# mayataka/robotoc

Measured on AMD Instinct MI355X. Metric: riccati_sweeps_per_sec, higher is better.
Workload: dtype f64; 1 GPU; anymal_trot_N40 (nv=18,nu=12, 47 grids: 2 lifts + 2 impacts, switching constraints ns=6), 4096 DISTINCT OCP instances per GPU (randomised stage data and dx0), backward+forward Riccati sweep; per_gpu_batch=4096, stages=47, parallelism=instances sharded, dp1

## Files before the change

### robotoc_amd/csrc/riccati_backward_rv.hpp

```cpp
#pragma once
#include "riccati_backward.hpp"

namespace rtoc {

template <int NV, int NU>
struct RvCfg {
  static constexpr int NX = 2 * NV;
  static constexpr int T = (NX + 15) / 16;
  static constexpr int LDP = lds_ld(NX);
  static constexpr int KG = (NX + 3) / 4;
  static constexpr int KSU = (NU + 3) / 4;
  static constexpr int SCOL = NX - 16 * (T - 1);
  static constexpr int G0 = NV / 4;
  static constexpr int GS = 4 * (T - 1) + SCOL / 4;
  static constexpr bool STRIP4 = (SCOL == 4);
  static constexpr bool OK = (NX + NU == 16 * T) && (NX % 4 == 0) && (NU % 4 == 0) && (SCOL % 4 == 0) && (SCOL >= 1) &&
                             ((NV * NU) % 2 == 0) && (LDP % 2 == 0);
  static constexpr int HL = LDP / 2;
  static constexpr int NCH_A = NX * HL;
  static constexpr int PA = (NCH_A + 63) / 64;
  static constexpr int OFF_A = 0;
  static constexpr int OFF_ST = NX * LDP;
  static constexpr int CB = NV * NU / 2, CG = NU * NU / 2;
  static constexpr int pad8(int n) { return (n + 7) & ~7; }
// ... 22 lines not shown
#else
  return *p;
#endif
}
__device__ __forceinline__ void rv_st(double* p, double v) {
#if RTOC_RV_NT
  __builtin_nontemporal_store(v, p);
#else
  *p = v;
#endif
}
constexpr int RV_DMA_AUX = RTOC_RV_NT ? 2 : 0;

template <int N>
__device__ __forceinline__ double dpp_from_right(double v) {
  const int lo = __builtin_amdgcn_update_dpp(0, __double2loint(v), 0x100 + N, 0xF, 0xF, true);
  const int hi = __builtin_amdgcn_update_dpp(0, __double2hiint(v), 0x100 + N, 0xF, 0xF, true);
  return __hiloint2double(hi, lo);
}
template <int N>
__device__ __forceinline__ double dpp_from_left(double v) {
  const int lo = __builtin_amdgcn_update_dpp(0, __double2loint(v), 0x110 + N, 0xF, 0xF, true);
  const int hi = __builtin_amdgcn_update_dpp(0, __double2hiint(v), 0x110 + N, 0xF, 0xF, true);
  return __hiloint2double(hi, lo);
}

constexpr int rv_dpp_ctrl(int from) { return from > 0 ? 0x100 + from : (from < 0 ? 0x110 - from : 0xE4); }
template <int R>
__device__ __forceinline__ double d4_to_c(double d0, double d1) {
  int h[2];
#pragma unroll
  for (int e = 0; e < 2; ++e) {
    const int a0 = e ? __double2hiint(d0) : __double2loint(d0), a1 = e ? __double2hiint(d1) : __double2loint(d1);
    const int x = __builtin_amdgcn_update_dpp(0, a0, rv_dpp_ctrl(4 * R), 0xF, 0x1, true);
    h[e] = __builtin_amdgcn_update_dpp(x, a1, rv_dpp_ctrl(4 * R - 4), 0xF, 0x2, true);
  }
  return __hiloint2double(h[1], h[0]);
}

__host__ __device__ constexpr int rv_tile_row(int T, int n) {
  int k = 0;
  for (int c = 0; c < T; ++c)
    for (int t = c + 1; t < T; ++t) {
      if (k == n) return c;
      ++k;
    }
  return n - k;
}
__host__ __device__ constexpr int rv_tile_col(int T, int n) {
  int k = 0;
  for (int c = 0; c < T; ++c)
    for (int t = c + 1; t < T; ++t) {
      if (k == n) return t;
      ++k;
    }
  return n - k;
}

__device__ __forceinline__ void rv_lds_sync() {
  asm volatile("s_waitcnt lgkmcnt(0)" ::: "memory");
  __builtin_amdgcn_wave_barrier();
}

#ifdef RTOC_ENABLE_PROF
#define RV_PROF(k)                                                                                        \
  do {                                                                                                    \
    if (a.prof && b == 0 && lane0 == 0) a.prof[st * 32 + (k)] = (long long)__builtin_readcyclecounter(); \
  } while (0)
#else
#define RV_PROF(k) do { } while (0)
#endif

template <int NV, int NU, int NS, bool SA, bool STO = false>
__global__ __launch_bounds__(64, 2) void riccati_backward_rv_kernel(BwdArgs a) {
  using C = RvCfg<NV, NU>;
  static_assert(C::OK, "shape does not fill the tiles of the stacked operand");
  constexpr int NP_ = NV - NU;
  static_assert(!SA || (NV % 16 == 2 && C::T == 3 && NP_ > 0 && NP_ <= 8 && NP_ % 2 == 0),
                "structured form: the lane shift of the c-part is NV mod 16 = 2, corner columns in tiles 0 and 1");
  constexpr int NX = C::NX, T = C::T, LDP = C::LDP, KG = C::KG, KSU = C::KSU, SCOL = C::SCOL, G0 = C::G0, GS = C::GS;
  constexpr bool STRIP4 = C::STRIP4 && !STO && RTOC_RV_MERGE_PBT;
  constexpr int RS = SCOL / 4;
  constexpr rtoc_layout SL = StaticLayout<NV, NU, NS>::make();
  constexpr rtoc_record_layout KL = SL.kkt, RL = SL.ric;
  constexpr int VOFF_LX = KL.off[RTOC_KKT_LX] - KL.off[RTOC_KKT_FX], VOFF_LU = KL.off[RTOC_KKT_LU] - KL.off[RTOC_KKT_FX];
  static_assert(VOFF_LX > 0 && VOFF_LU > VOFF_LX && VOFF_LX % 2 == 0 && VOFF_LU % 2 == 0, "Fx, lx, lu lie behind one another in the record");
  static_assert(KL.off[RTOC_KKT_FXX] % 2 == 0 && KL.off[RTOC_KKT_FVU] % 2 == 0 && KL.off[RTOC_KKT_QUU] % 2 == 0 && KL.off[RTOC_KKT_FX] % 2 == 0 &&
                    KL.stride % 2 == 0, "16-byte chunks");
  constexpr int VOFF_FFX = KL.off[RTOC_KKT_FFX] - KL.off[RTOC_KKT_FX], VOFF_HX = KL.off[RTOC_KKT_HX] - KL.off[RTOC_KKT_FX],
                VOFF_HU = KL.off[RTOC_KKT_HU] - KL.off[RTOC_KKT_FX], VOFF_SCAL = KL.off[RTOC_KKT_SCAL] - KL.off[RTOC_KKT_FX];
  static_assert(!STO || (VOFF_FFX > VOFF_LU && VOFF_HX > VOFF_FFX && VOFF_HU > VOFF_HX && VOFF_SCAL > VOFF_HU && VOFF_SCAL % 2 == 0), "fx, hx, hu, scalars behind lu");
  static_assert(!STO || SCOL + 2 < 16, "two more rider lanes in the last column tile");
  static_assert(!STO || SCOL >= 3, "lanes 0..2 of the G product are idle (the controls are shifted by SCOL lanes)");
  constexpr int CB = C::CB, CG = C::CG, CV = STO ? (VOFF_SCAL + 8) / 2 : (VOFF_LU + NU + 1) / 2, NCH_S = CB + CG + CV, PS = (NCH_S + 63) / 64;
  constexpr int ST_BV = C::OFF_ST, ST_G = ST_BV + 2 * CB, ST_FX = ST_G + 2 * CG, ST_LX = ST_FX + VOFF_LX, ST_LU = ST_FX + VOFF_LU;
  constexpr int ST_FFX = ST_FX + VOFF_FFX, ST_HX = ST_FX + VOFF_HX, ST_HU = ST_FX + VOFF_HU, ST_SCAL = ST_FX + VOFF_SCAL;
  constexpr int NSCR = (STO || RTOC_RV_ONE_SCRATCH) ? 1 : 2;
  constexpr int OFF_Y = ST_FX + 2 * CV, OFF_LINV = OFF_Y + C::pad8(NU * NU), OFF_SCR = OFF_LINV + C::pad8(NU), SCR_LD = 17,
                SCR_TILE = C::pad8(16 * SCR_LD), LDS_DOUBLES = OFF_SCR + NSCR * SCR_TILE;
  static_assert(NU * NU <= NSCR * SCR_TILE, "the Cholesky factor is parked in the transpose scratch");
  static_assert(!STO || 2 * C::pad8(NX) + NX <= SCR_TILE, "s | Psi | Phi gathered in the scratch");
  constexpr int OFF_GRID = LDS_DOUBLES, GRID_INTS = 2 * (20 * 1024 / 8 - LDS_DOUBLES);
  static_assert(GRID_INTS >= 64, "room for the grid table");
  static_assert(LDS_DOUBLES * 8 <= 20 * 1024, "eight instances per CU");
  extern __shared__ __attribute__((aligned(16))) double smem[];
  double* const sA = smem + C::OFF_A;
  double* const sBv = smem + ST_BV;
  double* const sG = smem + ST_G;
  double* const sY = smem + OFF_Y;
  double* const scr = smem + OFF_SCR;

  const int b = a.first + (int)blockIdx.x;
  if (b >= a.batch) return;
  const int lane0 = threadIdx.x;
  int lane = lane0 & 63, li = lane & 15, q = lane >> 4;
  const int N = a.nstages - 1;
  const size_t kinst = (size_t)b * a.nstages * KL.stride;
  const size_t rinst = (size_t)b * a.nstages * RL.stride;
  const int hi = a.seg_hi, lo = a.seg_lo;
  unsigned stat = 0;
#ifdef RTOC_RV_DEBUG_MASK
  const int dbg = a.scan_ps_soff;
#define RV_DBG(bit) (dbg & (1 << (bit)))
#else
#define RV_DBG(bit) false
#endif

  auto issue_dma = [&](int stage) {
    const double* kp = a.kkt + kinst + (size_t)stage * KL.stride;
#pragma unroll
    for (int p = 0; p < PS; ++p) {
      const int n = lane + 64 * p;
      const int off = (n < CB) ? (KL.off[RTOC_KKT_FVU] + 2 * n)
                               : ((n < CB + CG) ? (KL.off[RTOC_KKT_QUU] + 2 * (n - CB)) : (KL.off[RTOC_KKT_FX] + 2 * (n - CB - CG)));
      if (64 * (p + 1) <= NCH_S || n < NCH_S)
        __builtin_amdgcn_global_load_lds(kp + off, (lds_ptr_t)(smem + C::OFF_ST + 128 * p), 16, 0, RV_DMA_AUX);
    }
    constexpr int CPP = 64 / C::HL, NPC = (NX + CPP - 1) / CPP;
    const unsigned col0 = (unsigned)lane / C::HL, ch0 = (unsigned)lane - col0 * C::HL;
    const unsigned voff = col0 * NX + ((ch0 < NX / 2) ? 2 * ch0 : 0);
    if (col0 < CPP) {
#pragma unroll
      for (int p = 0; p < NPC; ++p) {
        const double* kpp = kp + KL.off[RTOC_KKT_FXX] + p * CPP * NX;
        if ((p + 1) * CPP <= NX || p * CPP + (int)col0 < NX)
          __builtin_amdgcn_global_load_lds(kpp + voff, (lds_ptr_t)(sA + p * CPP * LDP), 16, 0, RV_DMA_AUX);
      }
    }
  };
  double hq[T][KSU];
  auto issue_hq = [&](int stage) {
    const double* kp = a.kkt + kinst + (size_t)stage * KL.stride + KL.off[RTOC_KKT_QXU];
#pragma unroll
    for (int c = 0; c < T; ++c)
#pragma unroll
      for (int ks = 0; ks < KSU; ++ks) {
        const int x = 16 * c + li, u = 4 * ks + q;
        hq[c][ks] = rv_ld(kp + ((x < NX) ? x : NX - 1) + u * NX);
      }
  };

  d4 pp[T][T];
  double sv[KG];
  {
    const bool term = (hi == N - 1);
    const double* psrc = term ? (a.kkt + kinst + (size_t)N * KL.stride + KL.off[RTOC_KKT_QXX])
                              : (a.ric + rinst + (size_t)(hi + 1) * RL.stride + RL.off[RTOC_RIC_P]);
    const double* ssrc = term ? (a.kkt + kinst + (size_t)N * KL.stride + KL.off[RTOC_KKT_LX])
                              : (a.ric + rinst + (size_t)(hi + 1) * RL.stride + RL.off[RTOC_RIC_S]);
#pragma unroll
    for (int kt = 0; kt < T; ++kt)
#pragma unroll
      for (int mt = 0; mt < T; ++mt)
#pragma unroll
        for (int r = 0; r < 4; ++r) {
          const int i = 16 * kt + 4 * r + q, j = 16 * mt + li;
          const bool ok = i < NX && j < NX;
          const double v = psrc[ok ? i + j * NX : 0];
          pp[kt][mt][r] = ok ? v : 0.0;
        }
#pragma unroll
    for (int g = 0; g < KG; ++g) {
      const double v = ssrc[4 * g + q];
      sv[g] = (li == SCOL) ? (term ? -v : v) : 0.0;
    }
    if (term) {
      double* rr = a.ric + rinst + (size_t)N * RL.stride;
      const d2* s2 = reinterpret_cast<const d2*>(psrc);
      d2* t2 = reinterpret_cast<d2*>(rr + RL.off[RTOC_RIC_P]);
      for (int e = lane; e < NX * NX / 2; e += 64) t2[e] = s2[e];
      if (lane < NX) rr[RL.off[RTOC_RIC_S] + lane] = -ssrc[lane];
    }
  }
  issue_dma(hi);
  int* const sGrid = reinterpret_cast<int*>(smem + OFF_GRID);
  for (int e = lane; e < a.nstages; e += 64)
    sGrid[e] = (a.grid[e].type & 15) | ((a.grid[e].sto != 0) << 4) | ((a.grid[e].sto_next != 0) << 5) | (a.grid[e].dims << 8);
  double sc[5] = {0.0, 0.0, 0.0, 0.0, 0.0};
  auto phase_transition = [&](int pol, bool has_next) __attribute__((always_inline)) {
    double* pr = a.ric + rinst + (size_t)pol * RL.stride;
    const double xi = sc[0], chi = sc[1], rho = sc[2], eta = sc[3], iota = sc[4];
    double isg = 0.0;
    if (has_next) {
      double sgm = xi - 2.0 * chi + rho;
      const double eps = 1.4901161193847656e-08;
      if ((sgm * a.max_dts0) < fabs(eta - iota) || sgm < eps) sgm = fabs(sgm) + fabs(eta - iota) / a.max_dts0;
      isg = 1.0 / sgm;
    }
#pragma unroll
    for (int g = 0; g < KG; ++g) {
      const double v = sv[g];
      const double r1 = dpp_from_right<1>(v), r2 = dpp_from_right<2>(v), l1 = dpp_from_left<1>(v);
      const double d = (li == SCOL) ? (r1 - r2) : (l1 - v);
      double nv = 0.0;
      if (li == SCOL) nv = has_next ? __builtin_fma(isg * (eta - iota), d, v) : v;
      if (li == SCOL + 2) nv = has_next ? __builtin_fma(-isg * (xi - chi), d, l1) : l1;
      sv[g] = (li >= SCOL && li <= SCOL + 2) ? nv : 0.0;
      if (has_next && li == SCOL) pr[RL.off[RTOC_RIC_DTSDX] + 4 * g + q] = -isg * d;
    }
    sc[0] = 0.0, sc[1] = 0.0, sc[3] = 0.0;
    if (has_next) {
      if (lane0 == 0) {
        pr[RL.off[RTOC_RIC_SCAL] + RTOC_RIC_SCAL_DTSDTS] = isg * (xi - chi);
        pr[RL.off[RTOC_RIC_SCAL] + RTOC_RIC_SCAL_DTS0] = -isg * (eta - iota);
      }
      sc[2] = xi - isg * (xi - chi) * (xi - chi);
      sc[4] = eta - isg * (xi - chi) * (eta - iota);
    } else {
      sc[2] = xi;
      sc[4] = eta;
    }
  };
  rv_lds_sync();

  for (int st = hi; st >= lo; --st) {
    lane = lane0;
    asm volatile("" : "+v"(lane));
    lane &= 63;
    li = lane & 15;
    q = lane >> 4;
    const int gword = __builtin_amdgcn_readfirstlane(sGrid[st]);
    const bool impact = (gword & 15) == RTOC_GRID_IMPACT;
    const bool sto = STO && ((gword >> 4) & 1), sto_next = STO && ((gword >> 5) & 1);
    const int ns = impact ? 0 : (gword >> 8);
    const double* kr = a.kkt + kinst + (size_t)st * KL.stride;
    double* rr = a.ric + rinst + (size_t)st * RL.stride;
    if constexpr (STO) {
      const bool next_lift = (__builtin_amdgcn_readfirstlane(sGrid[st + 1]) & 15) == RTOC_GRID_LIFT;
      const bool prev_sto = st > 0 && ((__builtin_amdgcn_readfirstlane(sGrid[st > 0 ? st - 1 : 0]) >> 4) & 1);
      bool do_pt = false;
      int pol = st;
      if (impact) {
        do_pt = prev_sto || sto;
      } else if (next_lift) {
        do_pt = sto || sto_next;
        pol = st + 1;
      }
      if (do_pt) phase_transition(pol, sto_next);
      if (!impact && !sto_next) {
#pragma unroll
        for (int g = 0; g < KG; ++g) sv[g] = (li == SCOL + 2) ? 0.0 : sv[g];
      }
    }
    RV_PROF(0);
    if (st < hi)
      asm volatile("s_waitcnt vmcnt(1)" ::: "memory");
    else
      asm volatile("s_waitcnt vmcnt(0)" ::: "memory");
    RV_PROF(1);
    if constexpr (SA) {
      if (a.check_fxx) {
        const int j = (lane < NX) ? lane : 0;
        const double* colp = sA + j * LDP;
        int cnt_s = 0, cnt_c = 0;
#pragma unroll
        for (int i = 0; i < NV; i += 2) {
          const d2 v = *reinterpret_cast<const d2*>(colp + i);
#pragma unroll
          for (int e = 0; e < 2; ++e) {
            if (i + e < NP_) cnt_c += (v[e] != 0.0) ? 1 : 0;
            else cnt_s += (v[e] != 0.0) ? 1 : 0;
          }
        }
        const bool on_a = j >= NP_ && j < NV, on_c = j >= NV + NP_;
        const double want = on_a ? sA[NP_ + NP_ * LDP] : (on_c ? sA[NP_ + (NV + NP_) * LDP] : 0.0);
        const double got = colp[on_a ? j : (on_c ? j - NV : NP_)];
        const bool corner_col = j < NP_ || (j >= NV && j < NV + NP_);
        const int allowed = ((on_a || on_c) && got != 0.0) ? 1 : 0;
        const bool bad = ((on_a || on_c) && got != want) || cnt_s != allowed || (!corner_col && cnt_c != 0);
        if (lane < NX && bad) stat |= RTOC_STAT_FXX_UNSTRUCTURED;
      }
    }

    if (!RV_DBG(4)) issue_hq(st);
    d4 f[T][T];
    if (RV_DBG(0)) {
#pragma unroll
      for (int c = 0; c < T; ++c)
#pragma unroll
        for (int t = c; t < T; ++t) f[c][t] = zero4();
    } else {
      const double* qb_ = kr + KL.off[RTOC_KKT_QXX];
      const unsigned lic = (li < SCOL) ? li : SCOL - 1;
      const unsigned vx = q + li * NX, vxl = q + lic * NX;
      const unsigned vt = li + q * NX, vtl = lic + q * NX;
#pragma unroll
      for (int c = 0; c < T; ++c)
#pragma unroll
        for (int t = c; t < T; ++t)
#pragma unroll
          for (int r = 0; r < 4; ++r) {
            if (16 * c + 4 * r >= NX) {
              f[c][t][r] = 0.0;
              continue;
            }
            const double vt_ = rv_ld(qb_ + ((t < T - 1) ? vt : vtl) + (16 * t + (16 * c + 4 * r) * NX));
            if (t == c) {
              f[c][t][r] = vt_;
            } else {
              const double v = rv_ld(qb_ + ((t < T - 1) ? vx : vxl) + (16 * c + 4 * r + 16 * t * NX));
              f[c][t][r] = 0.5 * (v + vt_);
            }
          }
    }

    RV_PROF(2);
    d4 acc[T];
    double bts[KSU];
#pragma unroll
    for (int c = 0; c < T; ++c) acc[c] = zero4();
#pragma unroll
    for (int ks = 0; ks < KSU; ++ks) bts[ks] = 0.0;
    if (!impact) {
#pragma unroll
      for (int g = G0; g < KG; ++g) {
        const int k = 4 * g + q - NV, u = li - SCOL;
        const bool ok = k >= 0 && u >= 0;
        const double v = sBv[ok ? k + u * NV : 0];
        const double bv = ok ? v : 0.0;
#pragma unroll
        for (int c = 0; c < T; ++c) acc[c] = mfma16(pp[g / 4][c][g % 4], bv, acc[c]);
      }
      d4 gacc = zero4();
#pragma unroll
      for (int g = G0; g < KG; ++g) {
        const int k = 4 * g + q - NV;
        const bool ok = k >= 0 && li < NU;
        const double v = sBv[ok ? k + li * NV : 0];
        const double av = ok ? v : 0.0;
        const double srow = dpp_from_right<SCOL>(sv[g]);
        const double bv = (li < (STO ? 3 : 1)) ? srow : acc[g / 4][g % 4];
        gacc = mfma16(av, bv, gacc);
      }
#pragma unroll
      for (int r = 0; r < KSU; ++r) {
        const int u0 = q + 4 * r, u1 = li - SCOL;
        if (u0 < NU && u1 >= 0) sG[u0 + u1 * NU] += gacc[r];
        bts[r] = gacc[r];
      }
    }
    RV_PROF(3);
#if RTOC_RV_MERGE_PBT
#pragma unroll
    for (int g = 0; g < KG; ++g) pp[g / 4][T - 1][g % 4] = (li >= SCOL) ? acc[g / 4][g % 4] : pp[g / 4][T - 1][g % 4];
#endif
    RV_PROF(4);
    if (!impact) {
      rv_lds_sync();
      if (wave_llt_inv<NU, NU, 16, false>(sG, scr, smem + OFF_LINV, sY, NU, lane)) stat |= RTOC_STAT_QUU_NOT_SPD;
      rv_lds_sync();
    }

    RV_PROF(5);
    double xd[6] = {0.0, 0.0, 0.0, 0.0, 0.0, 0.0};
    double hT[T][KSU];
    double lup[KSU];
#pragma unroll
    for (int ks = 0; ks < KSU; ++ks) lup[ks] = 0.0;
#pragma unroll
    for (int t = 0; t < T; ++t) {
      d4 w[T];
#pragma unroll
      for (int tm = 0; tm < T; ++tm) w[tm] = zero4();
#pragma unroll
      for (int ks = 0; ks < KSU; ++ks) w[T - 1][RS + ks] = (impact || (t == T - 1 && li >= SCOL)) ? 0.0 : hq[t][ks];
      const double* pb_ = (t < T - 1 || li < SCOL) ? (sA + q + (16 * t + li) * LDP) : (smem + ((STO && li == SCOL + 1) ? ST_FFX : ST_FX) + q);
      const bool okb = (t < T - 1) || li <= SCOL || (STO && sto && !impact && li == SCOL + 1);
      auto group_dense = [](int g) { return 4 * g < NP_ || 4 * g + 3 >= NV; };
      auto row_dense = [&](int g) { return 4 * g + q < NP_ || 4 * g + q >= NV; };
      const bool sa_tile = SA && t < T - 1;
      if constexpr (STRIP4) {
        if (t == T - 1) {
          static_assert(!SA || NV + NP_ <= 16 * (T - 1), "the corner columns lie left of the last column tile");
          auto state_block_empty = [](int g) { return SA && 4 * g + 3 < NV && 4 * g + 3 + NV < 16 * (T - 1); };
          const int j4 = li & 3;
          const double* pbs = sA + q + (16 * (T - 1) + j4) * LDP;
          const double* pbr = smem + ST_FX + q;
          const double mr = (j4 == 0) ? 1.0 : 0.0;
          double ws4[T][2];
#pragma unroll
          for (int tm = 0; tm < T; ++tm) ws4[tm][0] = 0.0, ws4[tm][1] = 0.0;
          double bs4[2] = {0.0, 0.0}, br4[2];
          if (!state_block_empty(0)) bs4[0] = pbs[0];
          br4[0] = pbr[0];
#pragma unroll
          for (int g = 0; g < KG; ++g) {
            if (g + 1 < KG) {
              if (!state_block_empty(g + 1)) bs4[(g + 1) & 1] = pbs[4 * (g + 1)];
              br4[(g + 1) & 1] = pbr[4 * (g + 1)];
            }
            __builtin_amdgcn_sched_barrier(0);
            const double b0 = bs4[g & 1], b1 = mr * br4[g & 1];
#pragma unroll
            for (int tm = 0; tm < T; ++tm) {
              if (!state_block_empty(g)) ws4[tm][0] = mfma4(pp[g / 4][tm][g % 4], b0, ws4[tm][0]);
              ws4[tm][1] = mfma4(pp[g / 4][tm][g % 4], b1, ws4[tm][1]);
            }
            __builtin_amdgcn_sched_barrier(0);
          }
#pragma unroll
          for (int tm = 0; tm < T; ++tm) {
            const d4 cv = {d4_to_c<0>(ws4[tm][0], ws4[tm][1]), d4_to_c<1>(ws4[tm][0], ws4[tm][1]), d4_to_c<2>(ws4[tm][0], ws4[tm][1]),
                           d4_to_c<3>(ws4[tm][0], ws4[tm][1])};
#pragma unroll
            for (int r = 0; r < 4; ++r) w[tm][r] = (tm == T - 1 && r >= RS) ? w[tm][r] + cv[r] : cv[r];
          }
        }
      }
      double braw[2];
      braw[0] = pb_[0];
#pragma unroll
      for (int g = 0; g < (STRIP4 && t == T - 1 ? 0 : KG); ++g) {
        if (g + 1 < KG) braw[(g + 1) & 1] = pb_[4 * (g + 1)];
        __builtin_amdgcn_sched_barrier(0);
        const double bv = okb ? braw[g & 1] : 0.0;
        const double bm = (!sa_tile || row_dense(g)) ? bv : 0.0;
#pragma unroll
        for (int tm = 0; tm < T; ++tm) {
          double av = pp[g / 4][tm][g % 4];
#if !RTOC_RV_MERGE_PBT
          if (tm == T - 1) av = (li >= SCOL) ? acc[g / 4][g % 4] : av;
#endif
          if (sa_tile && tm < T - 1) {
            if (group_dense(g)) w[tm] = mfma16(av, bm, w[tm]);
          } else {
            w[tm] = mfma16(av, bv, w[tm]);
          }
        }
        __builtin_amdgcn_sched_barrier(0);
      }
      if (sa_tile) {
        const double ca = sA[NP_ + NP_ * LDP], cc = sA[NP_ + (NV + NP_) * LDP];
        const int j = 16 * t + li;
        const double ca_l = (j >= NP_ && j < NV) ? ca : 0.0;
        const double cc_l = (j >= NV + NP_ && li >= NV % 16) ? cc : 0.0;
#pragma unroll
        for (int tm = 0; tm < T - 1; ++tm)
#pragma unroll
          for (int r = 0; r < 4; ++r) {
            w[tm][r] = __builtin_fma(ca_l, pp[tm][t][r], w[tm][r]);
            if (t >= 1 && 16 * t + 15 >= NV + NP_) w[tm][r] = __builtin_fma(cc_l, dpp_from_left<NV % 16>(pp[tm][t - 1][r]), w[tm][r]);
          }
      }
      if (t == T - 1) {
        const double m_eq = (li == SCOL) ? 1.0 : 0.0, m_lt = (li < SCOL) ? 1.0 : 0.0, sgn_col = (li == SCOL) ? -1.0 : 1.0;
#pragma unroll
        for (int g = 0; g < KG; ++g) w[g / 4][g % 4] = __builtin_fma(sgn_col, w[g / 4][g % 4], sv[g]);
        if (!impact) {
#pragma unroll
          for (int ks = 0; ks < KSU; ++ks) {
            if constexpr (!STO) {
              const double luv = smem[ST_LU + 4 * ks + q];
              lup[ks] = luv - dpp_from_left<SCOL>(bts[ks]) + w[T - 1][RS + ks];
            } else {
              const double seed = smem[((li == SCOL + 1) ? ST_HU : ST_LU) + 4 * ks + q];
              const double sgn = (li == SCOL) ? -1.0 : 1.0;
              const double v = ((li == SCOL + 2) ? 0.0 : seed) + sgn * dpp_from_left<SCOL>(bts[ks]) + w[T - 1][RS + ks];
              lup[ks] = (li >= SCOL && li <= SCOL + 2) ? v : 0.0;
            }
          }
        }
#pragma unroll
        for (int g = 0; g < KG; ++g) {
          if constexpr (!STO) {
            const double lxv = smem[ST_LX + 4 * g + q];
            f[g / 4][T - 1][g % 4] = __builtin_fma(-m_eq, lxv, m_lt * f[g / 4][T - 1][g % 4]);
          } else {
            const double xv = smem[((li == SCOL + 1) ? ST_HX : ST_LX) + 4 * g + q];
            const double cf = (li == SCOL) ? -1.0 : ((li == SCOL + 1 && sto && !impact) ? 1.0 : 0.0);
            f[g / 4][T - 1][g % 4] = __builtin_fma(cf, xv, m_lt * f[g / 4][T - 1][g % 4]);
          }
        }
        if constexpr (STO) {
          double da = 0.0, db = 0.0, dc = 0.0;
#pragma unroll
          for (int g = 0; g < KG; ++g) {
            const double fxv = smem[ST_FFX + 4 * g + q], Fxv = smem[ST_FX + 4 * g + q];
            da = __builtin_fma(fxv, w[g / 4][g % 4], da);
            db = __builtin_fma(fxv, sv[g], db);
            dc = __builtin_fma(Fxv, sv[g], dc);
          }
          da += __shfl_xor(da, 16, 64), db += __shfl_xor(db, 16, 64), dc += __shfl_xor(dc, 16, 64);
          da += __shfl_xor(da, 32, 64), db += __shfl_xor(db, 32, 64), dc += __shfl_xor(dc, 32, 64);
          xd[0] = readlane_d(da, SCOL);
          xd[1] = readlane_d(da, SCOL + 1) - readlane_d(db, SCOL + 1);
          xd[2] = readlane_d(db, SCOL + 1);
          xd[3] = readlane_d(dc, SCOL + 1);
          xd[4] = readlane_d(db, SCOL + 2);
          xd[5] = readlane_d(dc, SCOL + 2);
        }
      }
      RV_PROF(6 + 2 * t);
      if (st < hi && !RV_DBG(1)) {
        double* pw = a.ric + rinst + (size_t)(st + 1) * RL.stride + RL.off[RTOC_RIC_P];
        const unsigned vst = li + q * NX;
#pragma unroll
        for (int mt = 0; mt < T; ++mt)
#pragma unroll
          for (int r = 0; r < 4; ++r) {
            const int i = 16 * t + 4 * r + q, j = 16 * mt + li;
            if (i < NX && j < NX) rv_st(pw + (vst + (16 * mt + (16 * t + 4 * r) * NX)), pp[t][mt][r]);
          }
      }
#pragma unroll
      for (int ks = 0; ks < KSU; ++ks) hT[t][ks] = w[T - 1][RS + ks];
      double araw[2][T];
      auto load_a = [&](int g, double (&d)[T]) {
#pragma unroll
        for (int c = 0; c <= t; ++c) d[c] = sA[q + 4 * g + (16 * c + ((STRIP4 && c == T - 1) ? (li & 3) : li)) * LDP];
      };
      if constexpr (!SA) {
      load_a(0, araw[0]);
#pragma unroll
      for (int g = 0; g < KG; ++g) {
        if (g + 1 < KG) load_a(g + 1, araw[(g + 1) & 1]);
        __builtin_amdgcn_sched_barrier(0);
        const double bw = w[g / 4][g % 4];
#pragma unroll
        for (int c = 0; c <= t; ++c) {
          if (STRIP4 && c == T - 1) {
            f[c][t][0] = mfma4(araw[g & 1][c], bw, f[c][t][0]);
            continue;
          }
          const double av = (c < T - 1 || li < SCOL) ? araw[g & 1][c] : 0.0;
          f[c][t] = mfma16(av, bw, f[c][t]);
        }
        __builtin_amdgcn_sched_barrier(0);
      }
      } else {
        constexpr int GFIRST = 0;
        static_assert(NP_ >= 1, "group 0 holds corner rows");
        auto next_dense = [&](int g) { int n = g + 1; while (n < KG && !group_dense(n)) ++n; return n; };
        load_a(GFIRST, araw[0]);
        int par = 0;
#pragma unroll
        for (int g = 0; g < KG; ++g) {
          if (!group_dense(g)) continue;
          const int gn = next_dense(g);
          if (gn < KG) load_a(gn, araw[par ^ 1]);
          __builtin_amdgcn_sched_barrier(0);
          const double bw = w[g / 4][g % 4];
          const bool corner_only = 4 * g + 3 < NV;
#pragma unroll
          for (int c = 0; c <= t; ++c) {
            if (corner_only && c == T - 1) continue;
            double av = (c < T - 1 || li < SCOL || STRIP4) ? araw[par][c] : 0.0;
            av = row_dense(g) ? av : 0.0;
            if (STRIP4 && c == T - 1) f[c][t][0] = mfma4(av, bw, f[c][t][0]);
            else f[c][t] = mfma16(av, bw, f[c][t]);
          }
          __builtin_amdgcn_sched_barrier(0);
          par ^= 1;
        }
        const double ca = sA[NP_ + NP_ * LDP], cc = sA[NP_ + (NV + NP_) * LDP];
#pragma unroll
        for (int c = 0; c <= t; ++c)
#pragma unroll
          for (int r = 0; r < 4; ++r) {
            const int gp = 4 * c + r;
            if (4 * gp + 3 >= NP_ && 4 * gp < NV) {
              const double coef = (4 * gp + q >= NP_ && 4 * gp + q < NV) ? ca : 0.0;
              f[c][t][r] = __builtin_fma(coef, w[c][r], f[c][t][r]);
            }
            if (4 * gp + 3 >= NV + NP_ && 4 * gp < NX) {
              constexpr int DHI = (NV - 2) / 4, DLO = (NV + 2) / 4;
              const int ghi = gp - DHI, glo = gp - DLO;
              const double hi_v = (ghi >= 0) ? w[(ghi >= 0 ? ghi : 0) / 4][(ghi >= 0 ? ghi : 0) % 4] : 0.0;
              const double lo_v = (glo >= 0) ? w[(glo >= 0 ? glo : 0) / 4][(glo >= 0 ? glo : 0) % 4] : 0.0;
              const double send = (q < 2) ? hi_v : lo_v;
              const double got = __shfl_xor(send, 32, 64);
              const double coef = (4 * gp + q >= NV + NP_) ? cc : 0.0;
              f[c][t][r] = __builtin_fma(coef, got, f[c][t][r]);
            }
          }
      }
      RV_PROF(7 + 2 * t);
    }

    double ksc[3] = {0.0, 0.0, 0.0};
    double scn[5] = {0.0, 0.0, 0.0, 0.0, 0.0};
    if constexpr (STO) {
      if (sto && !impact) {
        ksc[0] = smem[ST_SCAL + RTOC_KKT_SCAL_QTT], ksc[1] = smem[ST_SCAL + RTOC_KKT_SCAL_QTT_PREV], ksc[2] = smem[ST_SCAL + RTOC_KKT_SCAL_H];
#pragma unroll
        for (int g = 0; g < KG; ++g)
          if (li == SCOL + 1 || li == SCOL + 2) rr[((li == SCOL + 1) ? RL.off[RTOC_RIC_PSIX] : RL.off[RTOC_RIC_PHIX]) + 4 * g + q] = f[g / 4][T - 1][g % 4];
      }
    }
    asm volatile("s_waitcnt lgkmcnt(0)" ::: "memory");
    const bool dma_late = STO && NS > 0 && ns > 0;
    if (st > lo && !dma_late) {
      if (!RV_DBG(2)) issue_dma(st - 1);
    }
    asm volatile("" ::: "memory");

    RV_PROF(12);
    if (!impact) {
      d4 zt[T], kk[T];
      double y1[KSU], y2[KSU];
      double scm[3] = {0.0, 0.0, 0.0};
#pragma unroll
      for (int ks = 0; ks < KSU; ++ks) {
        const bool ok = li < NU;
        const double v1 = sY[(ok ? li : 0) + (4 * ks + q) * NU];
        const double v2 = sY[(4 * ks + q) + (ok ? li : 0) * NU];
// ... 320 lines not shown
```

### robotoc_amd/csrc/riccati_forward.hpp

```cpp
#pragma once
#include "device_utils.hpp"
#include "kernel_args.hpp"
#include "../../include/rtoc.h"

namespace rtoc {

#ifndef FWD_PREFETCH
#define FWD_PREFETCH 12
#endif
#ifndef FWD_WAVES_PER_SIMD
#define FWD_WAVES_PER_SIMD 2
#endif

template <int NV, int NU>
struct FwdPairCfg {
  static constexpr int NX = 2 * NV;
  static constexpr int G = 64 / NV;
  static constexpr int TX = (NX + G - 1) / G;
  static constexpr int TXP = (TX + 1) & ~1;
  static constexpr int TK = (NU + G - 1) / G;
  static constexpr int NVP = (NV + 1) & ~1;
  static constexpr int NF = NV * NU, NFP = (NF + 1) & ~1;
  static constexpr int TF = (NFP + 127) / 128;
};

template <int NWF>
__device__ __forceinline__ void fwd_sync() {
  if constexpr (NWF == 1)
    asm volatile("s_waitcnt lgkmcnt(0)" ::: "memory");
  else
    asm volatile("s_waitcnt lgkmcnt(0)\n\ts_barrier" ::: "memory");
}

template <int NV, int NU, int NS>
__global__ __launch_bounds__(64, FWD_WAVES_PER_SIMD) void riccati_forward_kernel(FwdArgs a) {
  using C = FwdPairCfg<NV, NU>;
  constexpr int NX = C::NX, G = C::G, TX = C::TX, TXP = C::TXP, TK = C::TK, NVP = C::NVP, NF = C::NF, TF = C::TF;
  constexpr int PF = FWD_PREFETCH < TX ? FWD_PREFETCH : TX;
  static_assert(NX + NU <= 64, "one lane per row of [Fxx; K] in the reductions");
  __shared__ __attribute__((aligned(16))) double sDx[2][NX + 8];
  __shared__ __attribute__((aligned(16))) double sXp[2][G * TXP];
  __shared__ __attribute__((aligned(16))) double sPa[G + 1][NX];
  __shared__ __attribute__((aligned(16))) double sPp[G + 1][NX];
  __shared__ __attribute__((aligned(16))) double sPk[NU + 1][NVP];
  __shared__ __attribute__((aligned(16))) double sF[TF * 128];
  __shared__ double sDu[NU + 8];
  __shared__ double sDt[NX];
  __shared__ double sRed[8];
  extern __shared__ int sGridTab[];
  const int tid = threadIdx.x;
  const int b = a.first + blockIdx.x;
  if (b >= a.batch) return;
  for (int st = tid; st < a.nstages; st += 64) {
    const rtoc_grid* gp = a.grid + st;
    sGridTab[st] = (gp->type & 15) | ((gp->sto != 0) << 4) | ((gp->sto_next != 0) << 5) |
                   ((gp->switching_constraint != 0) << 6) | (gp->dims << 8);
  }
  for (int e = tid; e < 2 * G * TXP; e += 64) (&sXp[0][0])[e] = 0.0;
  const int N = a.nstages - 1;
  constexpr rtoc_layout SL = StaticLayout<NV, NU, NS>::make();
  constexpr rtoc_record_layout KL = SL.kkt, RL = SL.ric, DL = SL.dir;
  const double* kb = a.kkt + (size_t)b * a.nstages * KL.stride;
  const double* rb = a.ric + (size_t)b * a.nstages * RL.stride;
  double* db = a.dir + (size_t)b * a.nstages * DL.stride;

  const bool lg = tid < G * NV;
  const int p = lg ? tid % NV : tid - G * NV;
  const int c = lg ? tid / NV : 0;
  const int cw = lg ? c : G;
  const bool xrow = tid < NX;
  const int r = xrow ? tid : NX - 1;
  const bool kl = tid >= NX && tid < NX + NU;
  const int u = kl ? tid - NX : 0;
  const int pos = (r % G) * TXP + r / G;
  __syncthreads();
  if (xrow) {
    const double v = a.dx0 ? a.dx0[(size_t)b * NX + tid] : db[DL.off[RTOC_DIR_DX] + tid];
    sDx[0][tid] = v;
    sXp[0][pos] = v;
    if (a.dx0) db[DL.off[RTOC_DIR_DX] + tid] = v;
  }
  __syncthreads();
  double dts = 0.0, dtsn = 0.0;
  {
    const rtoc_grid g0 = a.grid[0];
    if (g0.sto) {
      if (tid == 0) {
        double acc = 0.0;
        for (int k = 0; k < NX; ++k) acc += rb[RL.off[RTOC_RIC_DTSDX] + k] * sDx[0][k];
        sRed[0] = acc + rb[RL.off[RTOC_RIC_SCAL] + RTOC_RIC_SCAL_DTS0];
      }
      __syncthreads();
      dtsn = sRed[0];
      __syncthreads();
    }
  }
  const int lo = c * NX + 2 * p;
  auto moff = [&](int t) { return (NX % G == 0 || t < TX - 1 || G * t + c < NX) ? lo + t * (G * NX) : (NX - 1) * NX + 2 * p; };
  auto live = [&](int t) { return NX % G == 0 || t < TX - 1 || G * t + c < NX; };
  auto koff = [&](int t) { return (NU % G == 0 || t < TK - 1 || G * t + c < NU) ? lo + t * (G * NX) : (NU - 1) * NX + 2 * p; };
  auto klive = [&](int t) { return NU % G == 0 || t < TK - 1 || G * t + c < NU; };
  auto vec_ptr = [&](int st) {
    return xrow ? kb + (size_t)st * KL.stride + KL.off[RTOC_KKT_FX] + tid : rb + (size_t)st * RL.stride + RL.off[RTOC_RIC_KV] + u;
  };
  auto s_ptr = [&](int st) { return rb + (size_t)st * RL.stride + RL.off[RTOC_RIC_S] + r; };
  d2 fa[TX];
  double vec, sv;
#pragma unroll
  for (int t = 0; t < PF; ++t) fa[t] = *(const d2*)(kb + KL.off[RTOC_KKT_FXX] + moff(t));
  vec = *vec_ptr(0);
  sv = *s_ptr(0);
  int cur = 0;
  struct GridBits { int type, sto, sto_next, switching_constraint, dims; };
  for (int st = 0; st < N; ++st) {
    const int gb = __builtin_amdgcn_readfirstlane(sGridTab[st]);
    const GridBits g = {gb & 15, (gb >> 4) & 1, (gb >> 5) & 1, (gb >> 6) & 1, gb >> 8};
    const bool impact = g.type == RTOC_GRID_IMPACT, lift = g.type == RTOC_GRID_LIFT;
    const bool sto = g.sto != 0, sto_next = g.sto_next != 0;
    const double* kr = kb + (size_t)st * KL.stride;
    const double* rr = rb + (size_t)st * RL.stride;
    double* dr = db + (size_t)st * DL.stride;
    const double* dx = sDx[cur];
    const double* xp = sXp[cur];

    if (impact || lift) {
      dts = dtsn;
      dtsn = 0.0;
      if (lift && sto_next) {
        if (tid == 0) {
          double acc = 0.0;
          #pragma unroll 4
          for (int k = 0; k < NX; ++k) acc += rr[RL.off[RTOC_RIC_DTSDX] + k] * dx[k];
          acc += rr[RL.off[RTOC_RIC_SCAL] + RTOC_RIC_SCAL_DTS0];
          if (sto) acc += rr[RL.off[RTOC_RIC_SCAL] + RTOC_RIC_SCAL_DTSDTS] * dts;
          sRed[0] = acc;
        }
        fwd_sync<1>();
        dtsn = sRed[0];
        fwd_sync<1>();
      }
    }

    d2 fk[TK], ff[TF], fp[TX];
#pragma unroll
    for (int t = PF; t < TX; ++t) fa[t] = *(const d2*)(kr + KL.off[RTOC_KKT_FXX] + moff(t));
#pragma unroll
    for (int t = 0; t < TK; ++t) fk[t] = *(const d2*)(rr + RL.off[RTOC_RIC_K] + koff(t));
#pragma unroll
    for (int i = 0; i < TF; ++i) {
      const int e = 2 * (64 * i + tid);
      ff[i] = *(const d2*)(kr + KL.off[RTOC_KKT_FVU] + (e < NF ? e : 0));
    }
    double rd1 = 0.0, rd2 = 0.0, rd3 = 0.0, rdt = 0.0, rs0 = 0.0, rss = 0.0;
    if (sto) {
      rd1 = xrow ? kr[KL.off[RTOC_KKT_FFX] + tid] : rr[RL.off[RTOC_RIC_T] + u];
      rd2 = xrow ? rr[RL.off[RTOC_RIC_PSI] + tid] : rr[RL.off[RTOC_RIC_W] + u];
      rd3 = rr[RL.off[RTOC_RIC_PHI] + r];
    }
    if (impact && sto_next) {
      rdt = rr[RL.off[RTOC_RIC_DTSDX] + r];
      rs0 = rr[RL.off[RTOC_RIC_SCAL] + RTOC_RIC_SCAL_DTS0];
      rss = rr[RL.off[RTOC_RIC_SCAL] + RTOC_RIC_SCAL_DTSDTS];
    }
    d2 x[TXP / 2];
#pragma unroll
    for (int i = 0; i < TXP / 2; ++i) x[i] = *(const d2*)(xp + c * TXP + 2 * i);
    const d2 xq = *(const d2*)(dx + 2 * p);
    double a0 = 0.0, a1 = 0.0;
#pragma unroll
    for (int t = 0; t < TX; ++t) {
      const double xt = x[t / 2][t % 2];
      if (live(t)) {
        a0 += fa[t].x * xt;
        a1 += fa[t].y * xt;
      }
    }
    __builtin_amdgcn_sched_barrier(0);
#pragma unroll
    for (int t = 0; t < TX; ++t) fp[t] = *(const d2*)(rr + RL.off[RTOC_RIC_P] + moff(t));
    double pk[TK];
#pragma unroll
    for (int t = 0; t < TK; ++t) pk[t] = fk[t].x * xq.x + fk[t].y * xq.y;
#pragma unroll
    for (int i = 0; i < TF; ++i) *(d2*)(sF + 2 * (64 * i + tid)) = ff[i];
    double q0 = 0.0, q1 = 0.0;
#pragma unroll
    for (int t = 0; t < TX; ++t) {
      const double xt = x[t / 2][t % 2];
      if (live(t)) {
        q0 += fp[t].x * xt;
        q1 += fp[t].y * xt;
      }
    }
    double vec_n, sv_n;
    __builtin_amdgcn_sched_barrier(0);
    {
      const double* kn = kb + (size_t)(st + 1) * KL.stride;
#pragma unroll
      for (int t = 0; t < PF; ++t) fa[t] = *(const d2*)(kn + KL.off[RTOC_KKT_FXX] + moff(t));
      vec_n = *vec_ptr(st + 1);
      sv_n = *s_ptr(st + 1);
    }
    {
      d2 va = {a0, a1}, vp = {q0, q1};
      *(d2*)(&sPa[cw][2 * p]) = va;
      *(d2*)(&sPp[cw][2 * p]) = vp;
#pragma unroll
      for (int t = 0; t < TK; ++t) sPk[lg && klive(t) ? G * t + c : NU][p] = pk[t];
    }
    fwd_sync<1>();
    double acc_a = sPa[0][r], acc_p = sPp[0][r];
#pragma unroll
    for (int cc = 1; cc < G; ++cc) {
      acc_a += sPa[cc][r];
      acc_p += sPp[cc][r];
    }
    double kd = 0.0;
#pragma unroll 3
    for (int i = 0; i < NVP / 2; ++i) {
      const d2 w = *(const d2*)(&sPk[u][2 * i]);
      kd += w.x;
      if (2 * i + 1 < NV) kd += w.y;
    }
    if (kl && !impact) {
      double du = kd + vec;
      if (sto) {
        du += rd1 * (dtsn - dts);
        if (sto_next) du -= rd2 * dtsn;
      }
      sDu[u] = du;
      dr[DL.off[RTOC_DIR_DU] + u] = du;
    }
    fwd_sync<1>();
    double* dxn = sDx[cur ^ 1];
    if (xrow) {
      double v = vec + acc_a;
      if (!impact) {
        if (tid >= NV) {
#pragma unroll 4
          for (int cc = 0; cc < NU; ++cc) v += sF[cc * NV + tid - NV] * sDu[cc];
        }
        if (sto) v += rd1 * (dtsn - dts);
      }
      dxn[tid] = v;
      if (impact && sto_next) sDt[tid] = rdt;
      sXp[cur ^ 1][pos] = v;
      (dr + DL.stride)[DL.off[RTOC_DIR_DX] + tid] = v;
    }
    if (impact && sto_next) {
      fwd_sync<1>();
      if (tid == 0) {
        double acc = 0.0;
        #pragma unroll 4
        for (int k = 0; k < NX; ++k) acc += sDt[k] * dxn[k];
        acc += rs0;
        if (sto) acc += rss * dts;
        sRed[0] = acc;
      }
      fwd_sync<1>();
      dtsn = sRed[0];
    }
    if (xrow) {
      double lam = acc_p - sv;
      if (sto) {
        if (impact) {
          lam -= rd3 * dtsn;
        } else {
          lam += rd2 * (dtsn - dts);
          if (sto_next) lam -= rd3 * dtsn;
        }
      }
      dr[DL.off[RTOC_DIR_DLMDGMM] + tid] = lam;
    }
    if (NS > 0 && g.switching_constraint && tid < g.dims) {
      const double* M = rr + RL.off[RTOC_RIC_M] + tid;
      double acc = 0.0;
      #pragma unroll 4
      for (int j = 0; j < NX; ++j) acc += M[j * NS] * dx[j];
      acc += rr[RL.off[RTOC_RIC_MV] + tid];
      if (sto) {
        acc += rr[RL.off[RTOC_RIC_MT] + tid] * (dtsn - dts);
        if (sto_next) acc -= rr[RL.off[RTOC_RIC_MTN] + tid] * dtsn;
      }
      dr[DL.off[RTOC_DIR_DXI] + tid] = acc;
    }
    if (tid == 0) {
      dr[DL.off[RTOC_DIR_DTS] + 0] = dts;
      dr[DL.off[RTOC_DIR_DTS] + 1] = dtsn;
    }
    fwd_sync<1>();
    cur ^= 1;
    vec = vec_n;
    sv = sv_n;
  }
  {
    const double* rr = rb + (size_t)N * RL.stride;
    double* dr = db + (size_t)N * DL.stride;
    const double* xp = sXp[cur];
    d2 fp[TX], x[TXP / 2];
#pragma unroll
    for (int t = 0; t < TX; ++t) fp[t] = *(const d2*)(rr + RL.off[RTOC_RIC_P] + moff(t));
#pragma unroll
    for (int i = 0; i < TXP / 2; ++i) x[i] = *(const d2*)(xp + c * TXP + 2 * i);
    double q0 = 0.0, q1 = 0.0;
#pragma unroll
    for (int t = 0; t < TX; ++t) {
      const double xt = x[t / 2][t % 2];
      if (live(t)) {
        q0 += fp[t].x * xt;
        q1 += fp[t].y * xt;
      }
    }
    {
      d2 vp = {q0, q1};
      *(d2*)(&sPp[cw][2 * p]) = vp;
    }
    fwd_sync<1>();
    double acc_p = sPp[0][r];
#pragma unroll
    for (int cc = 1; cc < G; ++cc) acc_p += sPp[cc][r];
    if (xrow) dr[DL.off[RTOC_DIR_DLMDGMM] + tid] = acc_p - sv;
    if (tid == 0) {
      dr[DL.off[RTOC_DIR_DTS] + 0] = dts;
      dr[DL.off[RTOC_DIR_DTS] + 1] = dtsn;
    }
  }
}

template <int NV, int NU, int NS, int NWF>
__global__ __launch_bounds__(64 * NWF) void riccati_forward_mw_kernel(FwdArgs a) {
  constexpr int NX = 2 * NV, NT = 64 * NWF;
  static_assert(NX + NU <= NT, "one thread per row of [Fxx;K]");
  __shared__ double sDx[2][NX + 8];
  __shared__ double sDu[NU + 8];
  __shared__ double sRed[8];
  const int tid = threadIdx.x;
  const int b = a.first + blockIdx.x;
  if (b >= a.batch) return;
  const int N = a.nstages - 1;
  constexpr rtoc_layout SL = StaticLayout<NV, NU, NS>::make();
  constexpr rtoc_record_layout KL = SL.kkt, RL = SL.ric, DL = SL.dir;
  const double* kb = a.kkt + (size_t)b * a.nstages * KL.stride;
  const double* rb = a.ric + (size_t)b * a.nstages * RL.stride;
  double* db = a.dir + (size_t)b * a.nstages * DL.stride;

  if (tid < NX) {
    const double v = a.dx0 ? a.dx0[(size_t)b * NX + tid] : db[DL.off[RTOC_DIR_DX] + tid];
    sDx[0][tid] = v;
    if (a.dx0) db[DL.off[RTOC_DIR_DX] + tid] = v;
  }
  __syncthreads();
  double dts = 0.0, dtsn = 0.0;
  {
    const rtoc_grid g0 = a.grid[0];
    if (g0.sto) {
      if (tid == 0) {
        double acc = 0.0;
        for (int k = 0; k < NX; ++k) acc += rb[RL.off[RTOC_RIC_DTSDX] + k] * sDx[0][k];
        sRed[0] = acc + rb[RL.off[RTOC_RIC_SCAL] + RTOC_RIC_SCAL_DTS0];
      }
      __syncthreads();
      dtsn = sRed[0];
      __syncthreads();
    }
  }
  int cur = 0;
  for (int st = 0; st < N; ++st) {
    const rtoc_grid g = a.grid[st];
    const bool impact = g.type == RTOC_GRID_IMPACT, lift = g.type == RTOC_GRID_LIFT;
    const bool sto = g.sto != 0, sto_next = g.sto_next != 0;
    const double* kr = kb + (size_t)st * KL.stride;
    const double* rr = rb + (size_t)st * RL.stride;
    double* dr = db + (size_t)st * DL.stride;
    const double* dx = sDx[cur];
    double* dxn = sDx[cur ^ 1];

    if (impact || lift) {
      dts = dtsn;
      dtsn = 0.0;
      if (lift && sto_next) {
        if (tid == 0) {
          double acc = 0.0;
          for (int k = 0; k < NX; ++k) acc += rr[RL.off[RTOC_RIC_DTSDX] + k] * dx[k];
          acc += rr[RL.off[RTOC_RIC_SCAL] + RTOC_RIC_SCAL_DTS0];
          if (sto) acc += rr[RL.off[RTOC_RIC_SCAL] + RTOC_RIC_SCAL_DTSDTS] * dts;
          sRed[0] = acc;
        }
        __syncthreads();
        dtsn = sRed[0];
        __syncthreads();
      }
    }

    double acc_a = 0.0, acc_p = 0.0;
    if (tid < NX) {
      const double* A = kr + KL.off[RTOC_KKT_FXX] + tid;
      const double* P = rr + RL.off[RTOC_RIC_P] + tid;
#pragma unroll 18
      for (int j = 0; j < NX; ++j) {
        const double x = dx[j];
        acc_a += A[j * NX] * x;
        acc_p += P[j * NX] * x;
      }
    } else if (!impact && tid < NX + NU) {
      const int u = tid - NX;
      const double* K = rr + RL.off[RTOC_RIC_K] + (size_t)u * NX;
#pragma unroll 6
      for (int j = 0; j < NX; ++j) acc_a += K[j] * dx[j];
      double du = acc_a + rr[RL.off[RTOC_RIC_KV] + u];
      if (sto) {
        du += rr[RL.off[RTOC_RIC_T] + u] * (dtsn - dts);
        if (sto_next) du -= rr[RL.off[RTOC_RIC_W] + u] * dtsn;
      }
      sDu[u] = du;
      dr[DL.off[RTOC_DIR_DU] + u] = du;
    }
    __syncthreads();
    if (tid < NX) {
      double v = kr[KL.off[RTOC_KKT_FX] + tid] + acc_a;
      if (!impact) {
        if (tid >= NV) {
          const double* Bv = kr + KL.off[RTOC_KKT_FVU] + (tid - NV);
#pragma unroll 4
          for (int u = 0; u < NU; ++u) v += Bv[u * NV] * sDu[u];
        }
        if (sto) v += kr[KL.off[RTOC_KKT_FFX] + tid] * (dtsn - dts);
      }
      dxn[tid] = v;
      (dr + DL.stride)[DL.off[RTOC_DIR_DX] + tid] = v;
    }
    if (impact && sto_next) {
      __syncthreads();
      if (tid == 0) {
        double acc = 0.0;
        for (int k = 0; k < NX; ++k) acc += rr[RL.off[RTOC_RIC_DTSDX] + k] * dxn[k];
        acc += rr[RL.off[RTOC_RIC_SCAL] + RTOC_RIC_SCAL_DTS0];
        if (sto) acc += rr[RL.off[RTOC_RIC_SCAL] + RTOC_RIC_SCAL_DTSDTS] * dts;
        sRed[0] = acc;
      }
      __syncthreads();
      dtsn = sRed[0];
    }
    if (tid < NX) {
      double lam = acc_p - rr[RL.off[RTOC_RIC_S] + tid];
      if (sto) {
        if (impact) {
          lam -= rr[RL.off[RTOC_RIC_PHI] + tid] * dtsn;
        } else {
          lam += rr[RL.off[RTOC_RIC_PSI] + tid] * (dtsn - dts);
          if (sto_next) lam -= rr[RL.off[RTOC_RIC_PHI] + tid] * dtsn;
        }
      }
      dr[DL.off[RTOC_DIR_DLMDGMM] + tid] = lam;
    }
    if (NS > 0 && g.switching_constraint && tid < g.dims) {
      const double* M = rr + RL.off[RTOC_RIC_M] + tid;
      double acc = 0.0;
      for (int j = 0; j < NX; ++j) acc += M[j * NS] * dx[j];
      acc += rr[RL.off[RTOC_RIC_MV] + tid];
      if (sto) {
        acc += rr[RL.off[RTOC_RIC_MT] + tid] * (dtsn - dts);
        if (sto_next) acc -= rr[RL.off[RTOC_RIC_MTN] + tid] * dtsn;
      }
      dr[DL.off[RTOC_DIR_DXI] + tid] = acc;
    }
    if (tid == 0) {
      dr[DL.off[RTOC_DIR_DTS] + 0] = dts;
      dr[DL.off[RTOC_DIR_DTS] + 1] = dtsn;
    }
    __syncthreads();
    cur ^= 1;
  }
  {
    const double* rr = rb + (size_t)N * RL.stride;
    double* dr = db + (size_t)N * DL.stride;
    const double* dx = sDx[cur];
    if (tid < NX) {
      const double* P = rr + RL.off[RTOC_RIC_P] + tid;
      double acc = 0.0;
#pragma unroll 6
      for (int j = 0; j < NX; ++j) acc += P[j * NX] * dx[j];
      dr[DL.off[RTOC_DIR_DLMDGMM] + tid] = acc - rr[RL.off[RTOC_RIC_S] + tid];
    }
    if (tid == 0) {
      dr[DL.off[RTOC_DIR_DTS] + 0] = dts;
      dr[DL.off[RTOC_DIR_DTS] + 1] = dtsn;
    }
  }
}

template <int NV>
__global__ void unconstr_fill_kernel(FillArgs a) {
  constexpr int NX = 2 * NV;
  const int rec = blockIdx.x;
  if (rec >= a.batch * a.nstages) return;
  double* r = a.kkt + (size_t)rec * a.kl.stride;
  double* A = r + a.kl.off[RTOC_KKT_FXX];
  double* Bv = r + a.kl.off[RTOC_KKT_FVU];
  for (int e = threadIdx.x; e < NX * NX; e += blockDim.x) {
    const int i = e % NX, j = e / NX;
    double v = (i == j) ? 1.0 : 0.0;
    if (i < NV && j == i + NV) v = a.dt;
    A[e] = v;
  }
  for (int e = threadIdx.x; e < NV * NV; e += blockDim.x) {
    const int i = e % NV, j = e / NV;
    Bv[e] = (i == j) ? a.dt : 0.0;
  }
}

}
```

Measured before the change: 1.501 million sweeps/s.

## Exploit symmetry of Qxx and P to load only the upper triangle

```diff
diff --git a/robotoc_amd/csrc/riccati_backward_rv.hpp b/robotoc_amd/csrc/riccati_backward_rv.hpp
--- a/robotoc_amd/csrc/riccati_backward_rv.hpp
+++ b/robotoc_amd/csrc/riccati_backward_rv.hpp
@@ -348,7 +348,6 @@
     } else {
       const double* qb_ = kr + KL.off[RTOC_KKT_QXX];
       const unsigned lic = (li < SCOL) ? li : SCOL - 1;
-      const unsigned vx = q + li * NX, vxl = q + lic * NX;
       const unsigned vt = li + q * NX, vtl = lic + q * NX;
 #pragma unroll
       for (int c = 0; c < T; ++c)
@@ -360,13 +359,7 @@
               f[c][t][r] = 0.0;
               continue;
             }
-            const double vt_ = rv_ld(qb_ + ((t < T - 1) ? vt : vtl) + (16 * t + (16 * c + 4 * r) * NX));
-            if (t == c) {
-              f[c][t][r] = vt_;
-            } else {
-              const double v = rv_ld(qb_ + ((t < T - 1) ? vx : vxl) + (16 * c + 4 * r + 16 * t * NX));
-              f[c][t][r] = 0.5 * (v + vt_);
-            }
+            f[c][t][r] = rv_ld(qb_ + ((t < T - 1) ? vt : vtl) + (16 * t + (16 * c + 4 * r) * NX));
           }
     }
 
diff --git a/robotoc_amd/csrc/riccati_forward.hpp b/robotoc_amd/csrc/riccati_forward.hpp
--- a/robotoc_amd/csrc/riccati_forward.hpp
+++ b/robotoc_amd/csrc/riccati_forward.hpp
@@ -42,7 +42,7 @@
   __shared__ __attribute__((aligned(16))) double sXp[2][G * TXP];
   __shared__ __attribute__((aligned(16))) double sPa[G + 1][NX];
   __shared__ __attribute__((aligned(16))) double sPp[G + 1][NX];
-  __shared__ __attribute__((aligned(16))) double sPk[NU + 1][NVP];
+  __shared__ __attribute__((aligned(16))) double sPk[NX + NU + 1][NVP];
   __shared__ __attribute__((aligned(16))) double sF[TF * 128];
   __shared__ double sDu[NU + 8];
   __shared__ double sDt[NX];
@@ -100,6 +100,10 @@
   auto live = [&](int t) { return NX % G == 0 || t < TX - 1 || G * t + c < NX; };
   auto koff = [&](int t) { return (NU % G == 0 || t < TK - 1 || G * t + c < NU) ? lo + t * (G * NX) : (NU - 1) * NX + 2 * p; };
   auto klive = [&](int t) { return NU % G == 0 || t < TK - 1 || G * t + c < NU; };
+  const int pe = lg ? c - 2 * p : (1 << 20);
+  constexpr unsigned P_SILENT = 0x80000000u;
+  const auto prsrc = __builtin_amdgcn_make_buffer_rsrc(const_cast<double*>(rb), 0, a.nstages * (int)RL.stride * 8, 0x00020000);
+  const int prow = tid < NX + NU ? tid : NX + NU;
   auto vec_ptr = [&](int st) {
     return xrow ? kb + (size_t)st * KL.stride + KL.off[RTOC_KKT_FX] + tid : rb + (size_t)st * RL.stride + RL.off[RTOC_RIC_KV] + u;
   };
@@ -177,7 +181,10 @@
     }
     __builtin_amdgcn_sched_barrier(0);
 #pragma unroll
-    for (int t = 0; t < TX; ++t) fp[t] = *(const d2*)(rr + RL.off[RTOC_RIC_P] + moff(t));
+    for (int t = 0; t < TX; ++t) {
+      const unsigned vo = (pe + G * t <= 1) ? (unsigned)(lo + t * (G * NX)) * 8u : P_SILENT;
+      fp[t] = __builtin_bit_cast(d2, __builtin_amdgcn_raw_buffer_load_b128(prsrc, vo, (unsigned)(st * (int)RL.stride + (int)RL.off[RTOC_RIC_P]) * 8u, 0));
+    }
     double pk[TK];
 #pragma unroll
     for (int t = 0; t < TK; ++t) pk[t] = fk[t].x * xq.x + fk[t].y * xq.y;
@@ -187,10 +194,12 @@
 #pragma unroll
     for (int t = 0; t < TX; ++t) {
       const double xt = x[t / 2][t % 2];
-      if (live(t)) {
-        q0 += fp[t].x * xt;
-        q1 += fp[t].y * xt;
-      }
+      const int dd = pe + G * t;
+      const double o0 = q0 + fp[t].x * xt, o1 = q1 + fp[t].y * xt;
+      q0 = dd <= 0 ? o0 : q0;
+      q1 = dd <= 1 ? o1 : q1;
+      const double m1 = fp[t].y * xq.y, m01 = m1 + fp[t].x * xq.x;
+      sPk[lg && live(t) ? G * t + c : NX + NU][p] = dd < 0 ? m01 : (dd < 1 ? m1 : 0.0);
     }
     double vec_n, sv_n;
     __builtin_amdgcn_sched_barrier(0);
@@ -206,7 +215,7 @@
       *(d2*)(&sPa[cw][2 * p]) = va;
       *(d2*)(&sPp[cw][2 * p]) = vp;
 #pragma unroll
-      for (int t = 0; t < TK; ++t) sPk[lg && klive(t) ? G * t + c : NU][p] = pk[t];
+      for (int t = 0; t < TK; ++t) sPk[lg && klive(t) ? NX + G * t + c : NX + NU][p] = pk[t];
     }
     fwd_sync<1>();
     double acc_a = sPa[0][r], acc_p = sPp[0][r];
@@ -218,10 +227,11 @@
     double kd = 0.0;
 #pragma unroll 3
     for (int i = 0; i < NVP / 2; ++i) {
-      const d2 w = *(const d2*)(&sPk[u][2 * i]);
+      const d2 w = *(const d2*)(&sPk[prow][2 * i]);
       kd += w.x;
       if (2 * i + 1 < NV) kd += w.y;
     }
+    acc_p += xrow ? kd : 0.0;
     if (kl && !impact) {
       double du = kd + vec;
       if (sto) {
```

Result: faster. 1.609 million sweeps/s, median of 6 (+7.2%).
